# shayekh00/Knowledge_Distillation_for_Sensory_Substitution_in_Multimodal_Models

Measured on AMD Instinct MI355X. Metric: KD samples/sec/step (7B->0.5B, 336x336), higher is better.
Workload: dtype bf16; 1 GPU; c1: logit-based KD (LoCa, T=1), 7B->0.5B, 336x336; model=llava-onevision-qwen2-7b (teacher) -> 0.5b (student), global_batch=4, per_gpu_batch=4, seq_len=1536, image=336x336 (2 tiles, 1485 tokens), parallelism=dp1, teacher_lm_stream=bf16

## Files before the change

### include/kdstep.h

```cpp
#ifndef KDSTEP_H
#define KDSTEP_H

#include <stddef.h>
#include <stdint.h>

#ifdef __cplusplus
extern "C" {
#endif

typedef enum {
    KD_OK = 0,
    KD_ERR_SHAPE = 1,
    KD_ERR_DTYPE = 2,
    KD_ERR_ALIGN = 3,
    KD_ERR_ARCH = 4,
    KD_ERR_LABEL_RANGE = 5,
    KD_ERR_LAUNCH = 6,
    KD_ERR_ARG = 7,
    KD_ERR_WORKSPACE = 8
} kd_status;

int kd_abi_version(void);
const char* kd_last_error(void);
int kd_device_is_gfx950(int device);
// ... 79 lines not shown
    int32_t row_stats_top2;
    int32_t b_pretiled;
} kd_gemm_desc;

size_t kd_gemm_pretile_size(int N, int K, int glu);
int kd_gemm_pretile(const void* W, int64_t ldw, int N, int K, int glu, void* out, void* stream);
typedef struct kd_qkv_scatter {
    void* q; void* k; void* v;
    const float* cos_t; const float* sin_t;
    int32_t S, nq, nkv, hd, hdp;
} kd_qkv_scatter;

size_t kd_gemm_workspace_size(const kd_gemm_desc* desc);

int kd_gemm_plan(const kd_gemm_desc* desc, int32_t* variant, int32_t* split_k, int32_t* dp_tiles);

int kd_gemm(const kd_gemm_desc* desc, void* stream);

typedef struct {
    const void* q; const void* k; const void* v;
    void* o; float* lse;
    int32_t B, H, HKV, S, hd, hdp, causal;
} kd_attn_desc;
int kd_attn_fwd(const kd_attn_desc* desc, void* stream);

typedef struct {
    const void* q; const void* k; const void* v; const void* o; const void* dO;
    const float* lse; float* delta; float* dq; void* dk; void* dv;
    int32_t B, H, HKV, S, hd, hdp, causal;
    void* workspace; uint64_t workspace_bytes;
// ... 113 lines not shown
int kd_model_param_count(const kd_model_config* cfg);
int64_t kd_model_param_numel(const kd_model_config* cfg);
int kd_model_param_info(const kd_model_config* cfg, int index, char* name, int name_cap, int64_t* offset,
                        int64_t* numel, int64_t* rows, int64_t* cols);

int kd_anyres_batch_map(const int64_t* image_sizes_host, int B, int tiles, int32_t* map_host, int map_ld,
                        int32_t* len_host);

typedef struct kd_model kd_model;
int kd_model_create(const kd_model_config* cfg, const void* weights, float* grad, kd_model** out);
void kd_model_destroy(kd_model* m);
int kd_model_set_trainable(kd_model* m, int vision, int projector, int language);

int kd_model_set_residual_f32(kd_model* m, int vision, int language);

int64_t kd_model_fp8_scale_count(const kd_model* m);
int kd_model_quantize_fp8(const kd_model* m, void* q, float* scales, void* stream);
int kd_model_set_fp8(kd_model* m, const void* q, const float* scales);
typedef enum {
    KD_FP8_VISION = 1,
    KD_FP8_PROJECTOR = 2,
    KD_FP8_LM_ATTN = 4,
    KD_FP8_LM_MLP = 8,
    KD_FP8_LM_HEAD = 16,
    KD_FP8_ALL = 31
} kd_fp8_family;
int kd_model_set_fp8_families(kd_model* m, int families);

int kd_model_set_row_stats(kd_model* m, float* partials, int vs, float inv_t, int top2);

// ... 25 lines not shown
```

### knowledge_distillation_for_sensory_substitution_in_multimodal_models_amd/_native.py

```python
from __future__ import annotations

import ctypes as C
import os
from pathlib import Path

_PKG = Path(__file__).resolve().parent
LIB_PATH = Path(os.environ.get("KDSTEP_LIB", _PKG / "libkdstep.so"))
HEADER = _PKG.parent / "include" / "kdstep.h"

KD_OK = 0
ABI_VERSION = 9
STATUS_NAMES = {
    0: "KD_OK", 1: "KD_ERR_SHAPE", 2: "KD_ERR_DTYPE", 3: "KD_ERR_ALIGN", 4: "KD_ERR_ARCH",
    5: "KD_ERR_LABEL_RANGE", 6: "KD_ERR_LAUNCH", 7: "KD_ERR_ARG", 8: "KD_ERR_WORKSPACE",
}

KD_LOSS_NONE, KD_LOSS_LOCA, KD_LOSS_KL, KD_LOSS_KL_LOGTARGET = 0, 1, 2, 3


class KdLossParams(C.Structure):
    _fields_ = [
        ("variant", C.c_int32),
        ("temperature", C.c_float),
        ("alpha", C.c_float),
# ... 98 lines not shown
    "kd_last_error": (C.c_char_p, []),
    "kd_device_is_gfx950": (_i32, [_i32]),
    "kd_loss_workspace_size": (_sz, [_i32, _i32, _i32]),
    "kd_loss_fwd_bwd": (_i32, [_vp, _i64, _i32, _vp, _i64, _i32, _vp, _i32, _i32, KdLossParams,
                               _vp, _vp, _i64, _vp, _sz, _vp]),
    "kd_loss_check": (_i32, [_vp, _vp]),
    "kd_loss_student_stats": (_i32, [_vp, _i64, _i32, _i32, _f32, _vp, _vp]),
    "kd_gemm": (_i32, [C.POINTER(KdGemmDesc), _vp]),
    "kd_gemm_pretile_size": (_sz, [_i32, _i32, _i32]),
    "kd_gemm_pretile": (_i32, [_vp, _i64, _i32, _i32, _i32, _vp, _vp]),
    "kd_attn_fwd": (_i32, [C.POINTER(KdAttnDesc), _vp]),
    "kd_attn_bwd": (_i32, [C.POINTER(KdAttnBwdDesc), _vp]),
    "kd_attn_bwd_workspace_size": (C.c_size_t, [C.POINTER(KdAttnBwdDesc)]),
    "kd_gemm_workspace_size": (C.c_size_t, [C.POINTER(KdGemmDesc)]),
    "kd_gemm_plan": (_i32, [C.POINTER(KdGemmDesc), C.POINTER(_i32), C.POINTER(_i32), C.POINTER(_i32)]),
    "kd_norm_fwd": (_i32, [_i32, _vp, _i64, _vp, _vp, _vp, _i64, _vp, _vp, _i32, _i32, _f32, _i32, _vp]),
    "kd_norm_bwd_workspace_size": (_sz, [_i32, _i32]),
    "kd_norm_bwd": (_i32, [_i32, _vp, _i64, _vp, _vp, _i64, _vp, _vp, _vp, _i64, _i32, _vp, _vp, _i32, _vp, _sz,
                           _i32, _i32, _i32, _vp]),
    "kd_qkv_split": (_i32, [_vp, _i64, _vp, _vp, _vp, _vp, _vp, _i32, _i32, _i32, _i32, _i32, _i32, _vp]),
    "kd_qkv_merge": (_i32, [_vp, _vp, _vp, _vp, _i64, _vp, _vp, _i32, _i32, _i32, _i32, _i32, _i32, _vp]),
    "kd_swiglu_fwd": (_i32, [_vp, _i64, _vp, _i64, _i32, _i32, _vp]),
    "kd_swiglu_bwd": (_i32, [_vp, _i64, _vp, _i64, _vp, _i64, _i32, _i32, _vp]),
    "kd_act_bwd": (_i32, [_vp, _vp, _vp, _i64, _i32, _vp]),
    "kd_patchify": (_i32, [_vp, _i32, _vp, _i32, _i32, _i32, _i32, _vp]),
    "kd_embed_assemble": (_i32, [_vp, _vp, _vp, _vp, _vp, _vp, _i32, _i32, _i32, _vp, _vp]),
    "kd_image_src_map": (_i32, [_vp, _i32, _i32, _i64, _vp, _i32, _vp, _vp, _vp, _vp]),
    "kd_embed_bwd": (_i32, [_vp, _vp, _vp, _vp, _vp, _vp, _i32, _i32, _vp]),
    "kd_colsum": (_i32, [_vp, _i64, _i32, _i32, _vp, _i32, _vp]),
    "kd_row_group_mean": (_i32, [_vp, _i64, _i32, _i32, _i32, _vp, _vp]),
# ... 32 lines not shown
    "kd_gemv_gather_supported": (_i32, [_i32, _i32]),
    "kd_gemv_gather": (_i32, [_vp, _vp, _i64, _vp, _i32, _vp, _i32, _i32, _vp]),
    "kd_gemv_batch_gather": (_i32, [_vp, _i64, _i32, _vp, _i64, _vp, _i32, _vp, _i32, _i32, _vp]),
    "kd_gen_select_ids": (_i32, [_vp, _i64, _vp, _i32, _vp, _i32, _i32, _vp, _f32, _i32, _vp, _vp]),
    "kd_image_resize_u8": (_i32, [_vp, _i32, _i32, _vp, _i32, _i32, _vp, _sz, _vp]),
    "kd_anyres_tiles": (_i32, [_vp, _vp, _i32, _i32, _i32, _i32, _i32, _i32, _vp, _vp, _i32, _vp]),
    "kd_anyres_batch_map": (_i32, [_vp, _i32, _i32, _vp, _i32, _vp]),
    "kd_model_param_count": (_i32, [C.POINTER(KdModelConfig)]),
    "kd_model_param_numel": (_i64, [C.POINTER(KdModelConfig)]),
    "kd_model_param_info": (_i32, [C.POINTER(KdModelConfig), _i32, C.c_char_p, _i32, C.POINTER(_i64),
                                   C.POINTER(_i64), C.POINTER(_i64), C.POINTER(_i64)]),
    "kd_model_create": (_i32, [C.POINTER(KdModelConfig), _vp, _vp, C.POINTER(_vp)]),
    "kd_model_destroy": (None, [_vp]),
    "kd_model_set_trainable": (_i32, [_vp, _i32, _i32, _i32]),
    "kd_model_set_residual_f32": (_i32, [_vp, _i32, _i32]),
    "kd_model_fp8_scale_count": (_i64, [_vp]),
    "kd_model_quantize_fp8": (_i32, [_vp, _vp, _vp, _vp]),
    "kd_model_set_fp8": (_i32, [_vp, _vp, _vp]),
    "kd_model_set_fp8_families": (_i32, [_vp, _i32]),
    "kd_model_set_row_stats": (_i32, [_vp, _vp, _i32, _f32, _i32]),
    "kd_model_forward_workspace_size": (_sz, [_vp, _i32, _i32, _i32, _i32]),
    "kd_model_forward": (_i32, [_vp, _vp, _vp, _i32, _vp, _vp, _vp, _i32, _i32, _i32, _i32, _vp, _sz, _vp, _vp, _vp,
                                _vp, _vp, _vp, _vp]),
    "kd_model_backward_workspace_size": (_sz, [_vp, _i32, _i32, _i32]),
    "kd_model_backward": (_i32, [_vp, _vp, _vp, _vp, _vp, _vp, _i32, _i32, _i32, _vp, _vp, _vp, _sz, _vp, _vp,
                                 LAYER_CB, _vp]),
    "kd_timer_enable": (None, [_i32]),
    "kd_timer_count": (_i32, []),
    "kd_timer_read": (_i32, [_i32, C.c_char_p, _i32, C.POINTER(C.c_double), C.POINTER(_f32)]),
    "kd_timer_reset": (None, []),
# ... 40 lines not shown
```

### knowledge_distillation_for_sensory_substitution_in_multimodal_models_amd/csrc/abi.hip

```cpp
#include "common.h"
#include "launchers.h"
#include <cstring>

namespace kd {

static thread_local std::string g_last_error = "";

void set_error(const std::string& msg) { g_last_error = msg; }
int fail(int code, const std::string& msg) {
    g_last_error = msg;
    return code;
}

}

extern "C" {

int kd_abi_version(void) { return KD_ABI_VERSION; }

const char* kd_last_error(void) { return kd::g_last_error.c_str(); }

int kd_device_is_gfx950(int device) {
    hipDeviceProp_t prop;
    if (hipGetDeviceProperties(&prop, device) != hipSuccess) return 0;
// ... 13 lines not shown
int kd_loss_check(const void* workspace, void* stream) { return kd::kd_loss_check_impl(workspace, stream); }

int kd_loss_student_stats(const void* student_logits, int64_t ld_s, int V_s, int rows, float temperature,
                          float* stats_out, void* stream) {
    return kd::launch_kd_student_stats(student_logits, ld_s, V_s, rows, temperature, stats_out, stream);
}

int kd_gemm(const kd_gemm_desc* desc, void* stream) { return kd::gemm_timed(desc, stream); }
size_t kd_gemm_pretile_size(int N, int K, int glu) { return kd::gemm_pretile_size(N, K, glu); }
int kd_gemm_pretile(const void* W, int64_t ldw, int N, int K, int glu, void* out, void* stream) {
    return kd::launch_gemm_pretile(W, ldw, N, K, glu, out, stream);
}
size_t kd_gemm_workspace_size(const kd_gemm_desc* desc) { return kd::gemm_workspace_size(desc); }
int kd_gemm_plan(const kd_gemm_desc* desc, int32_t* variant, int32_t* split_k, int32_t* dp_tiles) {
    return kd::gemm_plan_query(desc, variant, split_k, dp_tiles);
}
int kd_attn_fwd(const kd_attn_desc* d, void* s) { return kd::launch_attn_fwd(d, s); }
int kd_attn_bwd(const kd_attn_bwd_desc* d, void* s) { return kd::launch_attn_bwd(d, s); }
size_t kd_attn_bwd_workspace_size(const kd_attn_bwd_desc* d) { return kd::attn_bwd_workspace_size(d); }
int kd_norm_fwd(int rms, const void* x, int64_t ldx, const void* w, const void* b, void* y, int64_t ldy, float* mean,
                float* rstd, int R, int D, float eps, int x_dtype, void* s) {
    KD_CHECK_ARG(x_dtype == KD_DTYPE_BF16 || x_dtype == KD_DTYPE_F32, "kd_norm_fwd: x_dtype");
    return kd::launch_norm_fwd(rms, x, ldx, w, b, y, ldy, mean, rstd, R, D, eps, s, x_dtype == KD_DTYPE_F32);
}
size_t kd_norm_bwd_workspace_size(int R, int D) { return kd::norm_bwd_ws(R, D); }
int kd_norm_bwd(int rms, const void* x, int64_t ldx, const void* w, const void* dy, int64_t lddy, const float* mean,
                const float* rstd, void* dx, int64_t lddx, int dx_accum, float* dw, float* db, int accum_w, void* ws,
                size_t wsb, int R, int D, int x_dtype, void* s) {
    KD_CHECK_ARG(x_dtype == KD_DTYPE_BF16 || x_dtype == KD_DTYPE_F32, "kd_norm_bwd: x_dtype");
    return kd::launch_norm_bwd(rms, x, ldx, w, dy, lddy, mean, rstd, dx, lddx, dx_accum, dw, db, accum_w, ws, wsb, R, D, s,
// ... 151 lines not shown
```

### knowledge_distillation_for_sensory_substitution_in_multimodal_models_amd/csrc/gemm.hip

```cpp
#include "common.h"

#include <cstring>
#include <type_traits>
#ifdef KD_AB_BUILD
#include <hipblaslt/hipblaslt.h>
#endif

namespace kd {
namespace {

constexpr int BM = 128, BN = 128, BK = 64, NTH = 256;
constexpr int TILE_BYTES = 128 * 64 * 2;
constexpr uint32_t OOB = 0x80000000u;

typedef __attribute__((address_space(3))) void lds_void_t;
typedef __attribute__((address_space(3))) bf16x4 lds_bf16x4_t;

struct GemmP {
    const bf16* A; const bf16* B; void* C;
    const void* bias; const bf16* resid; bf16* aux; const float* alpha_dev;
    int64_t lda, ldb, ldc, ldr, ld_aux;
    int M, N, K;
    float alpha;
    int c_f32, accumulate, bias_f32, act, res_mod;
// ... 1720 lines not shown
}
bool variant_known(int v) {
    const VariantInfo* i = variant_info(v);
#ifdef KD_AB_BUILD
    return i != nullptr;
#else
    return i && !i->ab;
#endif
}

bool sk_fits(int64_t tiles, int64_t nk, const kd_gemm_desc* d) {
    const int64_t dp = sk_dp_tiles(tiles, nk);
    return (tiles - dp) * nk >= 2 * SK_GRID && d->workspace && d->workspace_bytes >= sk_workspace_bytes(tiles - dp);
}

GemmPlan plan_gemm(const kd_gemm_desc* d, uint64_t ws_cap) {
    const int64_t M = d->M, N = d->N;
    const int64_t t256 = (int64_t)ceil_div(d->M, 256) * ceil_div(d->N, 256);
    const int64_t tiles[5] = {t256, (int64_t)ceil_div(d->M, 256) * ceil_div(d->N, 128),
                              (int64_t)ceil_div(d->M, 128) * ceil_div(d->N, 256), t256, t256};
    const bool kk = d->a_layout == KD_LAYOUT_K_MAJOR && d->b_layout == KD_LAYOUT_K_MAJOR;
    static const double step_c4[2][5] = {{0.8167, 0.5676, 0.5775, 0.7550, 0.7183}, {0.8016, 0.6139, 0.6026, 0.6942, 0.6876}};
    static const double fixed_c4[2][5] = {{8.830, 5.440, 5.343, 11.954, 5.888}, {9.291, 5.201, 5.162, 12.159, 8.442}};
    static const double step_c3[2][5] = {{0.7524, 0.5218, 0.5092, 0.6844, 0.7183}, {0.7375, 0.5501, 0.5469, 0.6022, 0.6876}};
    static const double fixed_c3[2][5] = {{5.253, 3.402, 3.414, 8.478, 5.888}, {5.885, 3.479, 3.398, 8.695, 8.442}};
    static const bool set3 = ab_knob("KD_PLAN_SET", 4) == 3;
    static const bool hybrid_on = ab_knob("KD_GEMM_HYBRID", 1) != 0;
    static const int split_cap = ab_knob("KD_SPLIT_CAP", 32);
    static const double split_pen = ab_knob("KD_SPLIT_PENALTY", 100) / 100.0;
    const double (&step_c)[2][5] = set3 ? step_c3 : step_c4;
    const double (&fixed_c)[2][5] = set3 ? fixed_c3 : fixed_c4;
    const double kBW = set3 ? 7.711e6 : 9.109e6;
    const double kSplitLaunch = set3 ? 5.623 : 6.499;
    constexpr bool kV9Auto = false;
    const double* step = step_c[kk ? 0 : 1];
    const double* fixed = fixed_c[kk ? 0 : 1];
    const int vcode[5] = {2, 3, 4, 16, 20};
    const int64_t nk = ceil_div(d->K, BK2);
    const VariantInfo* vi = variant_info(d->variant);
    const int fv = vi ? vi->cand : -1;
    const double out_e = (double)((d->c_dtype == KD_DTYPE_F32 ? 4 : 2) * (d->accumulate ? 2 : 1) +
                                  (d->residual ? (d->residual_dtype == KD_DTYPE_F32 ? 4 : 2) : 0) +
                                  (d->aux ? 2 : 0));
    const double out_b = (double)M * N * out_e;
    const int tbm[5] = {256, 256, 128, 256, 256}, tbn[5] = {256, 128, 256, 256, 256};
    GemmPlan best{fv >= 0 ? vcode[fv] : 2, 1, d->K, 0};
    double bt = 1e300;
    for (int v = 0; v < 5; ++v) {
        if (fv >= 0 && v != fv) continue;
        if (v == 4 && !kV9Auto && fv != 4) continue;
        for (int S = 1; S <= 32; ++S) {
// ... 49 lines not shown
    if (d->row_stats) return {Route::ROW_STATS, v8};
    if (d->act == KD_ACT_SWIGLU) {
        if (d->b_pretiled) return {Route::SWIGLU_PRETILED, v8};
        const bool sk = d->variant == 21 && sk_fits((int64_t)ceil_div(d->M, 256) * (d->N / 256), ceil_div(d->K, BK2), d);
        return {sk ? Route::SWIGLU_STREAMK : Route::SWIGLU, v8};
    }
    if (d->b_pretiled) return {Route::PRETILED, v8};
#ifdef KD_AB_BUILD
    if (d->variant == 30) return {Route::V8N, GemmPlan{30, 1, d->K, 0}};
#endif
    if (d->variant == 1 || !tiled_ok(d)) return {Route::V1, GemmPlan{1, 1, d->K, 0}};
    kd_gemm_desc d1 = *d;
    if (d->act == KD_ACT_DGELU_TANH || d->act == KD_ACT_DSWIGLU || d->qkv)
        d1.split_k = 1;
    return {Route::TILED, plan_gemm(&d1, d->workspace ? d->workspace_bytes : 0)};
}

GemmP make_params(const kd_gemm_desc* d) {
    GemmP p{};
    p.A = (const bf16*)d->A; p.B = (const bf16*)d->B; p.C = d->C;
    p.bias = d->bias; p.resid = (const bf16*)d->residual; p.aux = (bf16*)d->aux; p.alpha_dev = d->alpha_dev;
    p.lda = d->lda; p.ldb = d->ldb; p.ldc = d->ldc; p.ldr = d->ldr; p.ld_aux = d->ld_aux;
    p.M = d->M; p.N = d->N; p.K = d->K; p.alpha = d->alpha;
    p.c_f32 = d->c_dtype == KD_DTYPE_F32; p.accumulate = d->accumulate; p.bias_f32 = d->bias_dtype == KD_DTYPE_F32;
    p.act = d->act; p.res_mod = d->residual_row_mod;
    p.res_f32 = d->residual && d->residual_dtype == KD_DTYPE_F32;
    p.kchunk = d->K; p.gy = 1; p.rst_inv_t = 1.f;
    return p;
}

// ... 423 lines not shown
    }
    for (int i = n; i < GROUP_MAX; ++i) g.t0[i] = total;
    hipLaunchKernelGGL(k_gemm8_group, dim3((unsigned)total), dim3(NTH8), (gemm2_lds<256, 256>()), as_stream(stream_), g);
    KD_LAUNCH_CHECK("k_gemm8_group");
    return KD_OK;
}

int gemm_plan_query(const kd_gemm_desc* d, int32_t* var, int32_t* split, int32_t* dp) {
    KD_CHECK_ARG(d && var && split && dp, "gemm_plan: null pointer");
    KD_CHECK_SHAPE(d->M > 0 && d->N > 0 && d->K > 0, "gemm_plan: empty shape");
    const GemmPlan pl = gemm_route(d).plan;
    *var = pl.var; *split = pl.split; *dp = pl.dp_tiles;
    return KD_OK;
}

size_t gemm_workspace_size(const kd_gemm_desc* d) {
    if (!d || d->M <= 0 || d->N <= 0 || d->K <= 0 || d->variant == 1 || d->act == KD_ACT_SWIGLU) return 0;
    const GemmPlan pl = plan_gemm(d, ~0ull);
    if (pl.var == 21) return sk_workspace_bytes((int64_t)ceil_div(d->M, 256) * ceil_div(d->N, 256) - pl.dp_tiles);
    return pl.split > 1 ? (size_t)pl.split * d->M * d->N * 4 : 0;
}

}
```

### knowledge_distillation_for_sensory_substitution_in_multimodal_models_amd/csrc/launchers.h

```cpp
#pragma once
#include "common.h"

namespace kd {

int launch_kd_loss(const void* teacher, int64_t ld_t, int V_t, const void* student, int64_t ld_s,
                   int V_s, const int64_t* labels, int B, int L, kd_loss_params p, float* loss_out,
                   void* dlogits, int64_t ld_d, void* ws, size_t ws_bytes, void* stream);
size_t kd_loss_ws(int B, int L, int V);
int launch_kd_student_stats(const void* student, int64_t ld_s, int V_s, int rows, float temperature, float* out,
                            void* stream);
int kd_loss_check_impl(const void* ws, void* stream);
int launch_gemm(const kd_gemm_desc* d, void* stream);
int launch_gemm_group(const kd_gemm_desc* const* members, int n, void* stream);
bool gemm_group_member_ok(const kd_gemm_desc* d);
size_t gemm_workspace_size(const kd_gemm_desc* d);
size_t gemm_pretile_size(int N, int K, int glu);
int launch_gemm_pretile(const void* W, int64_t ldw, int N, int K, int glu, void* out, void* stream);
int gemm_plan_query(const kd_gemm_desc* d, int32_t* var, int32_t* split, int32_t* dp);
int launch_attn_fwd(const kd_attn_desc* d, void* stream);
int launch_attn_bwd(const kd_attn_bwd_desc* d, void* stream);
size_t attn_bwd_workspace_size(const kd_attn_bwd_desc* d);
int launch_norm_fwd(int rms, const void* x, int64_t ldx, const void* w, const void* b, void* y, int64_t ldy,
                    float* mean, float* rstd, int R, int D, float eps, void* stream, int x_f32 = 0);
size_t norm_bwd_ws(int R, int D);
int launch_norm_bwd(int rms, const void* x, int64_t ldx, const void* w, const void* dy, int64_t lddy, const float* mean,
                    const float* rstd, void* dx, int64_t lddx, int dx_accum, float* dw, float* db, int accum_w,
                    void* ws, size_t ws_bytes, int R, int D, void* stream, int x_f32 = 0, int dy_group = 0,
                    const void* dx_in = nullptr);
int launch_qkv_split(const void* qkv, int64_t ld, void* q, void* k, void* v, const float* cos_t, const float* sin_t,
                     int B, int S, int nq, int nkv, int hd, int hdp, void* stream);
int launch_qkv_merge(const float* dq, const void* dk, const void* dv, void* dqkv, int64_t ld, const float* cos_t,
                     const float* sin_t, int B, int S, int nq, int nkv, int hd, int hdp, void* stream);
int launch_swiglu_fwd(const void* gu, int64_t ldg, void* h, int64_t ldh, int M, int I, void* stream);
// ... 74 lines not shown
```

### knowledge_distillation_for_sensory_substitution_in_multimodal_models_amd/csrc/model.hip

```cpp
#include "common.h"
#include "launchers.h"

#include <algorithm>
#include <cmath>
#include <cstdlib>
#include <cstring>
#include <mutex>
#include <string>
#include <vector>

namespace kd {

namespace {
struct TimerRec {
    std::string key;
    double flops;
    hipEvent_t e0, e1;
};
std::mutex g_timer_mu;
std::vector<TimerRec> g_timer;
bool g_timer_on = false;
}

int gemm_timed(const kd_gemm_desc* d, void* stream) {
    if (!g_timer_on) return launch_gemm(d, stream);
    TimerRec r;
    const bool swiglu = d->act == KD_ACT_SWIGLU, f8 = d->ab_dtype == KD_DTYPE_FP8_E4M3;
    const bool dact = d->act == KD_ACT_DGELU_TANH || d->act == KD_ACT_DSWIGLU;
    r.key = swiglu ? std::string(f8 ? "gemm_f8_swiglu" : "gemm_kk_swiglu")
                   : (f8 ? std::string("gemm_f8") : std::string("gemm_") + (d->a_layout ? 'n' : 'k') + (d->b_layout ? 'n' : 'k') +
                                                        (dact ? "_dact" : ""));
    r.key += ":" + std::to_string(d->M) + "x" + std::to_string(d->N) + "x" + std::to_string(d->K) + ":" +
             (d->c_dtype == KD_DTYPE_F32 ? "f32" : "bf16") + (d->accumulate ? ":acc" : "");
    r.flops = 2.0 * d->M * d->N * d->K;
    (void)hipEventCreate(&r.e0);
    (void)hipEventCreate(&r.e1);
    (void)hipEventRecord(r.e0, as_stream(stream));
    const int st = launch_gemm(d, stream);
    (void)hipEventRecord(r.e1, as_stream(stream));
    std::lock_guard<std::mutex> g(g_timer_mu);
    g_timer.push_back(r);
    return st;
}

int gemm_group_timed(const kd_gemm_desc* const* ds, int n, void* stream) {
    if (!g_timer_on) return launch_gemm_group(ds, n, stream);
    TimerRec r;
    r.flops = 0;
// ... 124 lines not shown
enum LmField { LQW, LKW, LVW, LQB, LKB, LVB, LOW, LGW, LUW, LDW, LINW, LPOSTW, LNF };

}

}

struct kd_model {
    kd::Cfg C;
    std::vector<kd::Spec> specs;
    int64_t numel = 0;
    const kd::bf16* w = nullptr;
    float* g = nullptr;
    int train_vision = 0, train_projector = 0, train_language = 0;
    int lane_split_k = 0;
    int lane_group = 1, lane_v8_unsplit = 0;
    int rf32_v = 0, rf32_t = 0;
    std::vector<hipEvent_t> ev_pool;
    size_t ev_next = 0;
    const uint8_t* f8q = nullptr;
    const float* f8s = nullptr;
    std::vector<int64_t> soff;
    std::vector<int> fam;
    int f8_families = KD_FP8_ALL;
    float* rst = nullptr;
    int rst_vs = 0, rst_top2 = 0;
    float rst_inv_t = 1.f;
    int64_t n_scales = 0;
    int i_patch_w = 0, i_patch_b = 1, i_pos = 2, i_vis0 = 3, i_post_w, i_post_b, i_p1w, i_p1b, i_p2w, i_p2b, i_newline,
        i_embed, i_lm0, i_norm, i_head;

// ... 43 lines not shown
    const void* residual = nullptr;
    int64_t ldr = 0;
    void* aux = nullptr;
    int64_t ld_aux = 0;
    int residual_row_mod = 0;
    int accumulate = 0;
    int c_f32 = 0;
    int bias_f32 = 0;
    int split_k = 0;
    int res_f32 = 0;
    const kd_qkv_scatter* qkv = nullptr;
    float* row_stats = nullptr;
    int rs_vs = 0, rs_top2 = 0;
    float rs_inv_t = 1.f;
};

static const int g_split_default = ab_knob("KD_GEMM_SPLIT_K", 0);

int gemm(hipStream_t s, void* ws, int M, int N, int K, Op a, Op b, void* C, int64_t ldc, const GemmArgs& g) {
    kd_gemm_desc d;
    std::memset(&d, 0, sizeof(d));
    d.M = M; d.N = N; d.K = K;
    d.a_layout = a.layout; d.b_layout = b.layout;
    d.A = a.p; d.lda = a.ld; d.B = b.p; d.ldb = b.ld;
    d.C = C; d.ldc = ldc;
    d.c_dtype = g.c_f32 ? KD_DTYPE_F32 : KD_DTYPE_BF16;
    d.accumulate = g.accumulate;
    d.alpha = 1.f;
    d.bias = g.bias; d.bias_dtype = g.bias_f32 ? KD_DTYPE_F32 : KD_DTYPE_BF16;
    d.act = g.act;
    d.residual = g.residual; d.ldr = g.ldr;
    d.residual_dtype = g.res_f32 ? KD_DTYPE_F32 : KD_DTYPE_BF16;
    d.qkv = g.qkv;
    d.aux = g.aux; d.ld_aux = g.ld_aux;
    d.residual_row_mod = g.residual_row_mod;
    d.split_k = g.split_k ? g.split_k : g_split_default;
    if (d.split_k != 1 && ws) { d.workspace = ws; d.workspace_bytes = SPLITK_WS; }
    d.row_stats = g.row_stats; d.row_stats_vs = g.rs_vs; d.row_stats_inv_t = g.rs_inv_t; d.row_stats_top2 = g.rs_top2;
    return gemm_timed(&d, s);
}

static const bool g_fuse_dact = ab_knob("KD_FUSE_DACT", 1) != 0;
static bool fused_dact_ok(int64_t M, int64_t N) {
    return g_fuse_dact && M >= 128 && N >= 128 && N % 8 == 0 && M * N >= (int64_t)1 << 20;
}

#define KD_TRY(x)                    \
    do {                             \
        const int st__ = (x);        \
        if (st__ != KD_OK) return st__; \
    } while (0)

struct Lane {
    kd_model* m;
    hipStream_t main, lane;
    void* ws;
    void begin() {
        hipEvent_t e = m->event();
        (void)hipEventRecord(e, main);
        (void)hipStreamWaitEvent(lane, e, 0);
    }
    hipEvent_t end() {
        hipEvent_t e = m->event();
        (void)hipEventRecord(e, lane);
        return e;
    }
// ... 773 lines not shown
}

int kd_model_set_trainable(kd_model* m, int vision, int projector, int language) {
    KD_CHECK_ARG(m, "kd_model_set_trainable: null model");
    KD_CHECK_ARG(m->g || !(vision || projector || language), "kd_model_set_trainable: model has no grad buffer");
    m->train_vision = vision != 0;
    m->train_projector = projector != 0;
    m->train_language = language != 0;
    return KD_OK;
}

static bool fp8_stream_ok(bool f8, int fam, int rf32_v, int rf32_t) {
    return !f8 || ((!rf32_v || !(fam & KD_FP8_VISION)) && (!rf32_t || !(fam & (KD_FP8_LM_ATTN | KD_FP8_LM_MLP))));
}

int kd_model_set_residual_f32(kd_model* m, int vision, int language) {
    KD_CHECK_ARG(m, "kd_model_set_residual_f32: null model");
    KD_CHECK_ARG(fp8_stream_ok(m->f8q, m->f8_families, vision, language),
                 "kd_model_set_residual_f32: the tower's residual linears run in fp8 (bf16 residual only)");
    m->rf32_v = vision != 0;
    m->rf32_t = language != 0;
    return KD_OK;
}

int64_t kd_model_fp8_scale_count(const kd_model* m) { return m ? m->n_scales : -1; }

int kd_model_quantize_fp8(const kd_model* m, void* q, float* scales, void* stream) {
    KD_CHECK_ARG(m && q && scales, "kd_model_quantize_fp8: null pointer");
    KD_CHECK_ALIGN(q, 16, "kd_model_quantize_fp8: q must be 16-B aligned");
    for (size_t i = 0; i < m->specs.size(); ++i) {
// ... 45 lines not shown
    if (!m || B <= 0 || L <= 0 || n_tiles <= 0) return 0;
    return kd::plan_backward(m, B, L, n_tiles, nullptr).bytes;
}

int kd_model_forward(kd_model* m, const int64_t* ids, const void* pixels, int pixel_dtype, const int32_t* src,
                     const float* rope_cos, const float* rope_sin, int B, int L, int n_tiles, int save,
                     void* workspace, size_t workspace_bytes, void* hn, void* post_ln, void* logits,
                     void* const* kv_k, void* const* kv_v, int32_t* err, void* stream) {
    using namespace kd;
    KD_CHECK_ARG(m && ids && pixels && src && rope_cos && rope_sin && workspace && hn && err,
                 "kd_model_forward: null pointer");
    KD_CHECK_SHAPE(B > 0 && L > 0 && n_tiles > 0, "kd_model_forward: B, L, n_tiles must be positive");
    KD_CHECK_ARG(pixel_dtype == KD_DTYPE_BF16 || pixel_dtype == KD_DTYPE_F32, "kd_model_forward: pixel dtype");
    const FwdPlan P = plan_forward(m, B, L, n_tiles, save, workspace);
    KD_CHECK_ARG(workspace_bytes >= P.bytes, "kd_model_forward: workspace too small");
    const kd_model_config& c = m->C.c;
    hipStream_t s = as_stream(stream);
    const int NI = n_tiles, M = B * L, H = c.t_hidden;
    KD_TRY(vision_forward(m, P, pixels, pixel_dtype, NI, save, post_ln, s));
    {
        const int NT = NI * m->C.np(), D = c.v_hidden;
        GemmArgs g;
        g.bias = m->W(m->i_p1b);
        g.act = c.projector_act;
        g.aux = save ? P.ppre : nullptr;
        g.ld_aux = H;
        KD_TRY(lin(m, P, s, NT, H, D, P.x_vis_bf, D, m->i_p1w, P.z, H, g));
        GemmArgs g2;
        g2.bias = m->W(m->i_p2b);
        KD_TRY(lin(m, P, s, NT, H, H, P.z, H, m->i_p2w, P.feats, H, g2));
// ... 10 lines not shown
    return KD_OK;
}

int kd_model_backward(kd_model* m, const void* fwd_workspace, const int64_t* ids, const int32_t* src,
                      const float* rope_cos, const float* rope_sin, int B, int L, int n_tiles, const void* dhn,
                      const void* dpost, void* workspace, size_t workspace_bytes, void* stream, void* wgrad_stream,
                      kd_layer_cb on_layer_done, void* user) {
    using namespace kd;
    KD_CHECK_ARG(m && fwd_workspace && ids && src && rope_cos && rope_sin && dhn && workspace && wgrad_stream,
                 "kd_model_backward: null pointer");
    KD_CHECK_ARG(m->g, "kd_model_backward: the model has no grad buffer");
    KD_CHECK_SHAPE(B > 0 && L > 0 && n_tiles > 0, "kd_model_backward: B, L, n_tiles must be positive");
    const FwdPlan F = plan_forward(m, B, L, n_tiles, 1, const_cast<void*>(fwd_workspace));
    const BwdPlan P = plan_backward(m, B, L, n_tiles, workspace);
    KD_CHECK_ARG(workspace_bytes >= P.bytes, "kd_model_backward: workspace too small");
    const kd_model_config& c = m->C.c;
    hipStream_t s = as_stream(stream);
    Lane lane{m, s, as_stream(wgrad_stream), P.splitk_lane};
    hipEvent_t entry = m->event();
    (void)hipEventRecord(entry, lane.lane);
    const int NI = n_tiles, NT = NI * m->C.np(), M = B * L, H = c.t_hidden, D = c.v_hidden;
    const bf16* demb = nullptr;
    KD_TRY(lm_backward(m, F, P, rope_cos, rope_sin, B, L, dhn, lane, s, on_layer_done, user, &demb));
    wait(s, entry);
    const bool need_vision = m->train_vision != 0;
    KD_TRY(launch_embed_bwd(ids, src, demb, m->train_language ? m->G(m->i_embed) : nullptr, P.dfeats,
                            m->train_projector ? m->G(m->i_newline) : nullptr, M, H, s));
    {
        GemmArgs g0;
        KD_TRY(gemm(s, P.splitk_main, NT, H, H, km(P.dfeats, H), mn(m->W(m->i_p2w), H), P.dz, H, g0));
// ... 58 lines not shown
```

### knowledge_distillation_for_sensory_substitution_in_multimodal_models_amd/kd_module.py

```python
from __future__ import annotations

import contextlib
import inspect


import torch
import torch.nn as nn

from . import ops
from .dp import BackwardMarks, GradSync
from .modeling import (STREAM_PRIORITY_HIGH, STUDENT_05B, TEACHER_7B, LlavaOnevisionModel, real_width_config,
                       tiny_config)

try:
    import pytorch_lightning as _pl
    _Base = _pl.LightningModule
except Exception:
    class _Base(nn.Module):
        def __init__(self):
            super().__init__()
            self.logged = {}

        def log(self, name, value, **kw):
            self.logged[name] = value
# ... 168 lines not shown
        self.processor = processor
        self.model_name_student, self.model_name_teacher = model_name_student, model_name_teacher
        self.loss_group_size = loss_group_size
        self.accumulate_grad_batches = None if accumulate_grad_batches is None else int(accumulate_grad_batches)
        dev = _device()
        small = model_name_student not in _HUB_NAMES
        self.student_model = LlavaOnevisionModel(MODEL_CONFIGS[model_name_student], dev, trainable=True,
                                                 seed=seed_student, cpu_rng=small)
        self.teacher_model = None
        if self.uses_teacher:
            self.teacher_model = LlavaOnevisionModel(MODEL_CONFIGS[model_name_teacher], dev, trainable=False,
                                                     seed=seed_teacher, cpu_rng=small)
        if state_dict is not None:
            self.load_kd_state_dict(state_dict)
        self.config = self.student_model.cfg
        self._anchor = nn.Parameter(torch.zeros((), device=dev))
        self._stu_stream = torch.cuda.Stream(device=dev, priority=STREAM_PRIORITY_HIGH)
        self._opt_stream = self._stu_stream
        self.concurrent_student = True
        self._opt_done = torch.cuda.Event()
        self._opt_pending = False
        self._bwd_stream = self._stu_stream
        self._bwd_done = torch.cuda.Event()
        self._bwd_pending = False
        self.student_model.P.grad_fence = self._grad_fence
        self._ctx = None
        self._errors = _ErrorWatch(dev)
        self._errors.bind(self.student_model, self.teacher_model)
        self.keep_logits = False
        self.fuse_row_stats = False
# ... 261 lines not shown
    def kd_state_dict(self):
        if self._opt_pending:
            torch.cuda.current_stream().wait_event(self._opt_done)
        sd = {f"{self.ckpt_student_prefix}{k}": v for k, v in self.student_model.P.state_dict().items()}
        if self.teacher_model is not None:
            sd.update({f"teacher_model.{k}": v for k, v in self.teacher_model.P.state_dict().items()})
        return sd

    def load_kd_state_dict(self, sd):
        self.student_model.P.load_state_dict(sd, prefix=self.ckpt_student_prefix)
        if self.teacher_model is not None and any(k.startswith("teacher_model.") for k in sd):
            self.teacher_model.P.load_state_dict(sd, prefix="teacher_model.")
            if getattr(self.teacher_model, "fp8", False):
                self.teacher_model.enable_fp8(self.teacher_model.fp8_families)

    def load_hf_weights(self, student: dict | None = None, teacher: dict | None = None, strict: bool = True):
        if student is not None:
            self.student_model.load_hf_state_dict(student, strict=strict)
        if teacher is not None:
            if self.teacher_model is None:
                raise ValueError(f"{type(self).__name__} has no teacher")
            self.teacher_model.load_hf_state_dict(teacher, strict=strict)

    def _hparams(self):
        return {"model_name_student": self.model_name_student, "model_name_teacher": self.model_name_teacher,
                "learning_rate": self.learning_rate, "phase": self.phase, **self._run_hparams()}

    def _run_hparams(self):
        return {"loss_group_size": self.loss_group_size, "accumulate_grad_batches": self.accumulate_grad_batches,
                "teacher_fp8": getattr(self, "teacher_fp8", False),
# ... 104 lines not shown
```

### knowledge_distillation_for_sensory_substitution_in_multimodal_models_amd/modeling.py

```python
from __future__ import annotations

import ctypes as C
from dataclasses import dataclass, field

import numpy as np
import torch

from . import _native as NV
from . import anyres
from . import ops

IMAGE_TOKEN_ID = 151646


@dataclass(frozen=True)
class VisionConfig:
    hidden: int = 1152
    inter: int = 4304
    layers: int = 26
    heads: int = 16
    patch: int = 14
    image: int = 384
    eps: float = 1e-6

# ... 337 lines not shown
        self._ws = {}
        self.err = torch.zeros(1, dtype=torch.int32, device=self.device)
        self._train = [trainable] * 3
        self.wlane = WgradLane(self.device) if (trainable and self.device.type == "cuda") else None
        self._ncfg = native_config(cfg)
        if NV.lib().kd_model_param_numel(C.byref(self._ncfg)) != self.P.numel:
            raise RuntimeError("flat parameter layout differs from the library's (kd_model_param_info)")
        h = C.c_void_p()
        NV.call("kd_model_create", C.byref(self._ncfg), self.P.flat.data_ptr(),
                self.P.grad.data_ptr() if trainable else None, C.byref(h))
        self._h = h
        self.fp8 = False
        self.residual_f32 = (False, False)
        self.fp8_families = 0
        self.lm_stream_f32 = False
        self.set_residual_f32(*self._default_streams())

    def set_residual_f32(self, vision: bool, language: bool):
        NV.call("kd_model_set_residual_f32", self._h, int(vision), int(language))
        self.residual_f32 = (bool(vision), bool(language))
        self._ws = {}

    def __del__(self):
        h = getattr(self, "_h", None)
        if h is None or not h.value:
            return
        try:
            NV.lib().kd_model_destroy(h)
        except Exception:
            return
        self._h = None

    def set_trainable(self, vision: bool, projector: bool, language: bool):
        self._train = [bool(vision), bool(projector), bool(language)]
        NV.call("kd_model_set_trainable", self._h, *map(int, self._train))

# ... 170 lines not shown
```

### knowledge_distillation_for_sensory_substitution_in_multimodal_models_amd/ops.py

```python
from __future__ import annotations

import contextlib
import ctypes as C

import torch

from . import _native as NV

_WS: dict = {}


class KernelTimer:

    @property
    def enabled(self):
        return getattr(self, "_on", False)

    @enabled.setter
    def enabled(self, on):
        self._on = bool(on)
        NV.lib().kd_timer_enable(int(self._on))

    def reset(self):
        NV.lib().kd_timer_reset()
# ... 222 lines not shown
        _set_pretiled(d, b_pretiled, N, K, False)
    NV.call("kd_gemm", C.byref(d), _stream())
    return q, k, v


def gemm_plan(a: torch.Tensor, b: torch.Tensor, out: torch.Tensor | None = None, *, bias=None, act=None,
              residual=None, aux=None, alpha: float = 1.0, alpha_dev=None, accumulate: bool = False,
              out_dtype=torch.bfloat16, residual_row_mod: int = 0, variant: int = 0, split_k: int = 0):
    d = _gemm_desc(a, b, out, bias, act, residual, aux, alpha, alpha_dev, accumulate, out_dtype, residual_row_mod,
                   variant, split_k)[0]
    v, s_, dp = C.c_int32(), C.c_int32(), C.c_int32()
    NV.call("kd_gemm_plan", C.byref(d), C.byref(v), C.byref(s_), C.byref(dp))
    return v.value, s_.value, dp.value


_SPLIT_DEFAULT = [0]


@contextlib.contextmanager
def gemm_split_default(split_k: int):
    prev = _SPLIT_DEFAULT[0]
    _SPLIT_DEFAULT[0] = int(split_k)
    try:
        yield
    finally:
        _SPLIT_DEFAULT[0] = prev


def gemm(a: torch.Tensor, b: torch.Tensor, out: torch.Tensor | None = None, *, bias=None, act=None,
         residual=None, aux=None, alpha: float = 1.0, alpha_dev=None, accumulate: bool = False,
# ... 578 lines not shown
```

Measured before the change: 30.00 samples/s.

## Add CU-time GEMM planning objective for student training GEMMs

Adds a second GEMM planner objective that picks tile variant and split-K by total CU time rather than single-kernel latency, using the existing analytic cost model. The student model enables it by default for saved forward and backward passes, on the idea that student GEMMs run alongside the teacher and other streams, so CU occupancy matters more than isolated latency. This risks slower individual GEMMs when there is little concurrent work, and it relies on the accuracy of the cost model.

```diff
diff --git a/include/kdstep.h b/include/kdstep.h
--- a/include/kdstep.h
+++ b/include/kdstep.h
@@ -117,6 +117,11 @@
 size_t kd_gemm_workspace_size(const kd_gemm_desc* desc);
 
 int kd_gemm_plan(const kd_gemm_desc* desc, int32_t* variant, int32_t* split_k, int32_t* dp_tiles);
+
+typedef enum { KD_PLAN_LATENCY = 0, KD_PLAN_CU_TIME = 1 } kd_plan_objective;
+
+int kd_gemm_plan_objective(const kd_gemm_desc* desc, int objective, int32_t* variant, int32_t* split_k,
+                           int32_t* dp_tiles, double* latency_us, double* cu_us);
 
 int kd_gemm(const kd_gemm_desc* desc, void* stream);
 
@@ -260,6 +265,8 @@
 
 int kd_model_set_residual_f32(kd_model* m, int vision, int language);
 
+int kd_model_set_plan_objective(kd_model* m, int objective);
+
 int64_t kd_model_fp8_scale_count(const kd_model* m);
 int kd_model_quantize_fp8(const kd_model* m, void* q, float* scales, void* stream);
 int kd_model_set_fp8(kd_model* m, const void* q, const float* scales);
diff --git a/knowledge_distillation_for_sensory_substitution_in_multimodal_models_amd/_native.py b/knowledge_distillation_for_sensory_substitution_in_multimodal_models_amd/_native.py
--- a/knowledge_distillation_for_sensory_substitution_in_multimodal_models_amd/_native.py
+++ b/knowledge_distillation_for_sensory_substitution_in_multimodal_models_amd/_native.py
@@ -136,6 +136,8 @@
     "kd_attn_bwd_workspace_size": (C.c_size_t, [C.POINTER(KdAttnBwdDesc)]),
     "kd_gemm_workspace_size": (C.c_size_t, [C.POINTER(KdGemmDesc)]),
     "kd_gemm_plan": (_i32, [C.POINTER(KdGemmDesc), C.POINTER(_i32), C.POINTER(_i32), C.POINTER(_i32)]),
+    "kd_gemm_plan_objective": (_i32, [C.POINTER(KdGemmDesc), _i32, C.POINTER(_i32), C.POINTER(_i32), C.POINTER(_i32),
+                                      C.POINTER(C.c_double), C.POINTER(C.c_double)]),
     "kd_norm_fwd": (_i32, [_i32, _vp, _i64, _vp, _vp, _vp, _i64, _vp, _vp, _i32, _i32, _f32, _i32, _vp]),
     "kd_norm_bwd_workspace_size": (_sz, [_i32, _i32]),
     "kd_norm_bwd": (_i32, [_i32, _vp, _i64, _vp, _vp, _i64, _vp, _vp, _vp, _i64, _i32, _vp, _vp, _i32, _vp, _sz,
@@ -198,6 +200,7 @@
     "kd_model_destroy": (None, [_vp]),
     "kd_model_set_trainable": (_i32, [_vp, _i32, _i32, _i32]),
     "kd_model_set_residual_f32": (_i32, [_vp, _i32, _i32]),
+    "kd_model_set_plan_objective": (_i32, [_vp, _i32]),
     "kd_model_fp8_scale_count": (_i64, [_vp]),
     "kd_model_quantize_fp8": (_i32, [_vp, _vp, _vp, _vp]),
     "kd_model_set_fp8": (_i32, [_vp, _vp, _vp]),
diff --git a/knowledge_distillation_for_sensory_substitution_in_multimodal_models_amd/csrc/abi.hip b/knowledge_distillation_for_sensory_substitution_in_multimodal_models_amd/csrc/abi.hip
--- a/knowledge_distillation_for_sensory_substitution_in_multimodal_models_amd/csrc/abi.hip
+++ b/knowledge_distillation_for_sensory_substitution_in_multimodal_models_amd/csrc/abi.hip
@@ -51,6 +51,16 @@
 size_t kd_gemm_workspace_size(const kd_gemm_desc* desc) { return kd::gemm_workspace_size(desc); }
 int kd_gemm_plan(const kd_gemm_desc* desc, int32_t* variant, int32_t* split_k, int32_t* dp_tiles) {
     return kd::gemm_plan_query(desc, variant, split_k, dp_tiles);
+}
+int kd_gemm_plan_objective(const kd_gemm_desc* desc, int objective, int32_t* variant, int32_t* split_k, int32_t* dp_tiles,
+                           double* latency_us, double* cu_us) {
+    KD_CHECK_ARG(variant && split_k && dp_tiles && latency_us && cu_us, "kd_gemm_plan_objective: null pointer");
+    kd::GemmObjectivePlan pl;
+    const int st = kd::gemm_plan_objective_query(desc, objective, &pl);
+    if (st != KD_OK) return st;
+    *variant = pl.variant; *split_k = pl.split_k; *dp_tiles = pl.dp_tiles;
+    *latency_us = pl.latency_us; *cu_us = pl.cu_us;
+    return KD_OK;
 }
 int kd_attn_fwd(const kd_attn_desc* d, void* s) { return kd::launch_attn_fwd(d, s); }
 int kd_attn_bwd(const kd_attn_bwd_desc* d, void* s) { return kd::launch_attn_bwd(d, s); }
diff --git a/knowledge_distillation_for_sensory_substitution_in_multimodal_models_amd/csrc/gemm.hip b/knowledge_distillation_for_sensory_substitution_in_multimodal_models_amd/csrc/gemm.hip
--- a/knowledge_distillation_for_sensory_substitution_in_multimodal_models_amd/csrc/gemm.hip
+++ b/knowledge_distillation_for_sensory_substitution_in_multimodal_models_amd/csrc/gemm.hip
@@ -1,4 +1,5 @@
 #include "common.h"
+#include "launchers.h"
 
 #include <cstring>
 #include <type_traits>
@@ -1758,11 +1759,14 @@
     return (tiles - dp) * nk >= 2 * SK_GRID && d->workspace && d->workspace_bytes >= sk_workspace_bytes(tiles - dp);
 }
 
-GemmPlan plan_gemm(const kd_gemm_desc* d, uint64_t ws_cap) {
-    const int64_t M = d->M, N = d->N;
-    const int64_t t256 = (int64_t)ceil_div(d->M, 256) * ceil_div(d->N, 256);
-    const int64_t tiles[5] = {t256, (int64_t)ceil_div(d->M, 256) * ceil_div(d->N, 128),
-                              (int64_t)ceil_div(d->M, 128) * ceil_div(d->N, 256), t256, t256};
+struct PlanModel {
+    const double* step;
+    const double* fixed;
+    double kBW, kSplitLaunch, split_pen;
+    int split_cap;
+    bool hybrid_on;
+};
+PlanModel plan_model(const kd_gemm_desc* d) {
     const bool kk = d->a_layout == KD_LAYOUT_K_MAJOR && d->b_layout == KD_LAYOUT_K_MAJOR;
     static const double step_c4[2][5] = {{0.8167, 0.5676, 0.5775, 0.7550, 0.7183}, {0.8016, 0.6139, 0.6026, 0.6942, 0.6876}};
     static const double fixed_c4[2][5] = {{8.830, 5.440, 5.343, 11.954, 5.888}, {9.291, 5.201, 5.162, 12.159, 8.442}};
@@ -1776,9 +1780,20 @@
     const double (&fixed_c)[2][5] = set3 ? fixed_c3 : fixed_c4;
     const double kBW = set3 ? 7.711e6 : 9.109e6;
     const double kSplitLaunch = set3 ? 5.623 : 6.499;
+    return {step_c[kk ? 0 : 1], fixed_c[kk ? 0 : 1], kBW, kSplitLaunch, split_pen, split_cap, hybrid_on};
+}
+
+GemmPlan plan_gemm(const kd_gemm_desc* d, uint64_t ws_cap) {
+    const int64_t M = d->M, N = d->N;
+    const int64_t t256 = (int64_t)ceil_div(d->M, 256) * ceil_div(d->N, 256);
+    const int64_t tiles[5] = {t256, (int64_t)ceil_div(d->M, 256) * ceil_div(d->N, 128),
+                              (int64_t)ceil_div(d->M, 128) * ceil_div(d->N, 256), t256, t256};
+    const PlanModel pm = plan_model(d);
+    const double *step = pm.step, *fixed = pm.fixed;
+    const double kBW = pm.kBW, kSplitLaunch = pm.kSplitLaunch, split_pen = pm.split_pen;
+    const int split_cap = pm.split_cap;
+    const bool hybrid_on = pm.hybrid_on;
     constexpr bool kV9Auto = false;
-    const double* step = step_c[kk ? 0 : 1];
-    const double* fixed = fixed_c[kk ? 0 : 1];
     const int vcode[5] = {2, 3, 4, 16, 20};
     const int64_t nk = ceil_div(d->K, BK2);
     const VariantInfo* vi = variant_info(d->variant);
@@ -1858,6 +1873,55 @@
     if (d->act == KD_ACT_DGELU_TANH || d->act == KD_ACT_DSWIGLU || d->qkv)
         d1.split_k = 1;
     return {Route::TILED, plan_gemm(&d1, d->workspace ? d->workspace_bytes : 0)};
+}
+
+struct PlanCost { double latency_us, cu_us; };
+PlanCost plan_cost(const kd_gemm_desc* d, const GemmPlan& pl) {
+    const int v = pl.var == 2 ? 0 : pl.var == 3 ? 1 : pl.var == 4 ? 2 : pl.var == 16 ? 3 : pl.var == 20 ? 4 : -1;
+    if (v < 0) return {0, 0};
+    const int tbm[5] = {256, 256, 128, 256, 256}, tbn[5] = {256, 128, 256, 256, 256};
+    const PlanModel pm = plan_model(d);
+    const int64_t tiles = (int64_t)ceil_div(d->M, tbm[v]) * ceil_div(d->N, tbn[v]);
+    const int64_t nk = ceil_div(d->K, BK2), S = pl.split, kcs = S > 1 ? ceil_div(pl.kchunk, BK2) : nk;
+    const double whole = (double)nk * pm.step[v] + pm.fixed[v], part = (double)kcs * pm.step[v] + pm.fixed[v];
+    const double out_e = (double)((d->c_dtype == KD_DTYPE_F32 ? 4 : 2) * (d->accumulate ? 2 : 1) +
+                                  (d->residual ? (d->residual_dtype == KD_DTYPE_F32 ? 4 : 2) : 0) + (d->aux ? 2 : 0));
+    const int64_t dp = S > 1 ? pl.dp_tiles : 0, tail = tiles - dp;
+    const double elems = dp ? (double)tail * tbm[v] * tbn[v] : (double)d->M * d->N;
+    const double fold = S > 1 ? ((double)S * elems * 8 * pm.split_pen + elems * out_e) / pm.kBW + (dp ? 2 : 1) * pm.kSplitLaunch : 0;
+    const double lat = (double)(dp / 256) * whole + (double)((tail * S + 255) / 256) * part + fold;
+    const double cu = ((double)dp * whole + (double)tail * S * part) / 256 + fold;
+    return {lat, cu};
+}
+
+constexpr double kCuMargin = 0.05;
+
+GemmObjectivePlan plan_gemm_objective(const kd_gemm_desc* d, int objective) {
+    const GemmRoute r0 = gemm_route(d);
+    const PlanCost c0 = plan_cost(d, r0.plan);
+    const GemmObjectivePlan keep{r0.plan.var, r0.plan.split, r0.plan.dp_tiles, c0.latency_us, c0.cu_us, false};
+    const int fv = d->variant;
+    if (objective == 0 || r0.route != Route::TILED || !(fv == 0 || fv == 2 || fv == 3 || fv == 4 || fv == 16)) return keep;
+    GemmObjectivePlan best = keep;
+    bool found = false;
+    for (int code : {2, 3, 4, 16}) {
+        if (fv != 0 && code != fv) continue;
+        kd_gemm_desc df = *d;
+        df.variant = code;
+        df.split_k = d->split_k > 1 ? d->split_k : 1;
+        const GemmRoute r = gemm_route(&df);
+        if (r.route != Route::TILED || r.plan.var != code) continue;
+        const PlanCost c = plan_cost(&df, r.plan);
+        if (!found || c.cu_us < best.cu_us) {
+            best = GemmObjectivePlan{r.plan.var, r.plan.split, r.plan.dp_tiles, c.latency_us, c.cu_us, true};
+            found = true;
+        }
+    }
+    if (!found || best.cu_us > c0.cu_us) return keep;
+    if (best.variant == keep.variant && best.split_k == keep.split_k && best.dp_tiles == keep.dp_tiles) return keep;
+    const bool lat_is_candidate = r0.plan.dp_tiles == 0 && (r0.plan.split == 1 || d->split_k > 1);
+    if (lat_is_candidate && best.cu_us > c0.cu_us * (1.0 - kCuMargin)) return keep;
+    return best;
 }
 
 GemmP make_params(const kd_gemm_desc* d) {
@@ -2311,6 +2375,14 @@
     return KD_OK;
 }
 
+int gemm_plan_objective_query(const kd_gemm_desc* d, int objective, GemmObjectivePlan* out) {
+    KD_CHECK_ARG(d && out, "gemm_plan_objective: null pointer");
+    KD_CHECK_ARG(objective == KD_PLAN_LATENCY || objective == KD_PLAN_CU_TIME, "gemm_plan_objective: objective must be 0 or 1");
+    KD_CHECK_SHAPE(d->M > 0 && d->N > 0 && d->K > 0, "gemm_plan_objective: empty shape");
+    *out = plan_gemm_objective(d, objective);
+    return KD_OK;
+}
+
 size_t gemm_workspace_size(const kd_gemm_desc* d) {
     if (!d || d->M <= 0 || d->N <= 0 || d->K <= 0 || d->variant == 1 || d->act == KD_ACT_SWIGLU) return 0;
     const GemmPlan pl = plan_gemm(d, ~0ull);
diff --git a/knowledge_distillation_for_sensory_substitution_in_multimodal_models_amd/csrc/launchers.h b/knowledge_distillation_for_sensory_substitution_in_multimodal_models_amd/csrc/launchers.h
--- a/knowledge_distillation_for_sensory_substitution_in_multimodal_models_amd/csrc/launchers.h
+++ b/knowledge_distillation_for_sensory_substitution_in_multimodal_models_amd/csrc/launchers.h
@@ -17,6 +17,8 @@
 size_t gemm_pretile_size(int N, int K, int glu);
 int launch_gemm_pretile(const void* W, int64_t ldw, int N, int K, int glu, void* out, void* stream);
 int gemm_plan_query(const kd_gemm_desc* d, int32_t* var, int32_t* split, int32_t* dp);
+struct GemmObjectivePlan { int variant, split_k, dp_tiles; double latency_us, cu_us; bool forced; };
+int gemm_plan_objective_query(const kd_gemm_desc* d, int objective, GemmObjectivePlan* out);
 int launch_attn_fwd(const kd_attn_desc* d, void* stream);
 int launch_attn_bwd(const kd_attn_bwd_desc* d, void* stream);
 size_t attn_bwd_workspace_size(const kd_attn_bwd_desc* d);
diff --git a/knowledge_distillation_for_sensory_substitution_in_multimodal_models_amd/csrc/model.hip b/knowledge_distillation_for_sensory_substitution_in_multimodal_models_amd/csrc/model.hip
--- a/knowledge_distillation_for_sensory_substitution_in_multimodal_models_amd/csrc/model.hip
+++ b/knowledge_distillation_for_sensory_substitution_in_multimodal_models_amd/csrc/model.hip
@@ -20,6 +20,15 @@
 std::mutex g_timer_mu;
 std::vector<TimerRec> g_timer;
 bool g_timer_on = false;
+
+thread_local int t_plan_objective = KD_PLAN_LATENCY;
+struct PlanScope {
+    const int prev = t_plan_objective;
+    explicit PlanScope(int objective) { t_plan_objective = objective; }
+    ~PlanScope() { t_plan_objective = prev; }
+    PlanScope(const PlanScope&) = delete;
+    PlanScope& operator=(const PlanScope&) = delete;
+};
 }
 
 int gemm_timed(const kd_gemm_desc* d, void* stream) {
@@ -32,6 +41,10 @@
                                                         (dact ? "_dact" : ""));
     r.key += ":" + std::to_string(d->M) + "x" + std::to_string(d->N) + "x" + std::to_string(d->K) + ":" +
              (d->c_dtype == KD_DTYPE_F32 ? "f32" : "bf16") + (d->accumulate ? ":acc" : "");
+    if (t_plan_objective == KD_PLAN_CU_TIME) {
+        int32_t var = 0, split = 1, dp = 0;
+        if (gemm_plan_query(d, &var, &split, &dp) == KD_OK && split > 1) r.key += ":s" + std::to_string(split);
+    }
     r.flops = 2.0 * d->M * d->N * d->K;
     (void)hipEventCreate(&r.e0);
     (void)hipEventCreate(&r.e1);
@@ -186,6 +199,7 @@
     int train_vision = 0, train_projector = 0, train_language = 0;
     int lane_split_k = 0;
     int lane_group = 1, lane_v8_unsplit = 0;
+    int plan_objective = KD_PLAN_LATENCY;
     int rf32_v = 0, rf32_t = 0;
     std::vector<hipEvent_t> ev_pool;
     size_t ev_next = 0;
@@ -259,6 +273,12 @@
     int rs_vs = 0, rs_top2 = 0;
     float rs_inv_t = 1.f;
 };
+
+#define KD_TRY(x)                    \
+    do {                             \
+        const int st__ = (x);        \
+        if (st__ != KD_OK) return st__; \
+    } while (0)
 
 static const int g_split_default = ab_knob("KD_GEMM_SPLIT_K", 0);
 
@@ -282,6 +302,11 @@
     d.split_k = g.split_k ? g.split_k : g_split_default;
     if (d.split_k != 1 && ws) { d.workspace = ws; d.workspace_bytes = SPLITK_WS; }
     d.row_stats = g.row_stats; d.row_stats_vs = g.rs_vs; d.row_stats_inv_t = g.rs_inv_t; d.row_stats_top2 = g.rs_top2;
+    if (t_plan_objective == KD_PLAN_CU_TIME) {
+        GemmObjectivePlan pl;
+        KD_TRY(gemm_plan_objective_query(&d, KD_PLAN_CU_TIME, &pl));
+        if (pl.forced) { d.variant = pl.variant; d.split_k = pl.split_k; }
+    }
     return gemm_timed(&d, s);
 }
 
@@ -289,12 +314,6 @@
 static bool fused_dact_ok(int64_t M, int64_t N) {
     return g_fuse_dact && M >= 128 && N >= 128 && N % 8 == 0 && M * N >= (int64_t)1 << 20;
 }
-
-#define KD_TRY(x)                    \
-    do {                             \
-        const int st__ = (x);        \
-        if (st__ != KD_OK) return st__; \
-    } while (0)
 
 struct Lane {
     kd_model* m;
@@ -1098,6 +1117,14 @@
     return !f8 || ((!rf32_v || !(fam & KD_FP8_VISION)) && (!rf32_t || !(fam & (KD_FP8_LM_ATTN | KD_FP8_LM_MLP))));
 }
 
+int kd_model_set_plan_objective(kd_model* m, int objective) {
+    KD_CHECK_ARG(m, "kd_model_set_plan_objective: null model");
+    KD_CHECK_ARG(objective == KD_PLAN_LATENCY || objective == KD_PLAN_CU_TIME,
+                 "kd_model_set_plan_objective: objective must be KD_PLAN_LATENCY or KD_PLAN_CU_TIME");
+    m->plan_objective = objective;
+    return KD_OK;
+}
+
 int kd_model_set_residual_f32(kd_model* m, int vision, int language) {
     KD_CHECK_ARG(m, "kd_model_set_residual_f32: null model");
     KD_CHECK_ARG(fp8_stream_ok(m->f8q, m->f8_families, vision, language),
@@ -1173,6 +1200,7 @@
     KD_CHECK_ARG(pixel_dtype == KD_DTYPE_BF16 || pixel_dtype == KD_DTYPE_F32, "kd_model_forward: pixel dtype");
     const FwdPlan P = plan_forward(m, B, L, n_tiles, save, workspace);
     KD_CHECK_ARG(workspace_bytes >= P.bytes, "kd_model_forward: workspace too small");
+    const PlanScope plan_scope(save ? m->plan_objective : KD_PLAN_LATENCY);
     const kd_model_config& c = m->C.c;
     hipStream_t s = as_stream(stream);
     const int NI = n_tiles, M = B * L, H = c.t_hidden;
@@ -1213,6 +1241,7 @@
     const FwdPlan F = plan_forward(m, B, L, n_tiles, 1, const_cast<void*>(fwd_workspace));
     const BwdPlan P = plan_backward(m, B, L, n_tiles, workspace);
     KD_CHECK_ARG(workspace_bytes >= P.bytes, "kd_model_backward: workspace too small");
+    const PlanScope plan_scope(m->plan_objective);
     const kd_model_config& c = m->C.c;
     hipStream_t s = as_stream(stream);
     Lane lane{m, s, as_stream(wgrad_stream), P.splitk_lane};
diff --git a/knowledge_distillation_for_sensory_substitution_in_multimodal_models_amd/kd_module.py b/knowledge_distillation_for_sensory_substitution_in_multimodal_models_amd/kd_module.py
--- a/knowledge_distillation_for_sensory_substitution_in_multimodal_models_amd/kd_module.py
+++ b/knowledge_distillation_for_sensory_substitution_in_multimodal_models_amd/kd_module.py
@@ -206,6 +206,7 @@
         if state_dict is not None:
             self.load_kd_state_dict(state_dict)
         self.config = self.student_model.cfg
+        self.cu_time_plans = True
         self._anchor = nn.Parameter(torch.zeros((), device=dev))
         self._stu_stream = torch.cuda.Stream(device=dev, priority=STREAM_PRIORITY_HIGH)
         self._opt_stream = self._stu_stream
@@ -497,6 +498,14 @@
             if getattr(self.teacher_model, "fp8", False):
                 self.teacher_model.enable_fp8(self.teacher_model.fp8_families)
 
+    @property
+    def cu_time_plans(self) -> bool:
+        return self.student_model.plan_objective == 1
+
+    @cu_time_plans.setter
+    def cu_time_plans(self, on: bool):
+        self.student_model.set_plan_objective(1 if on else 0)
+
     def load_hf_weights(self, student: dict | None = None, teacher: dict | None = None, strict: bool = True):
         if student is not None:
             self.student_model.load_hf_state_dict(student, strict=strict)
diff --git a/knowledge_distillation_for_sensory_substitution_in_multimodal_models_amd/modeling.py b/knowledge_distillation_for_sensory_substitution_in_multimodal_models_amd/modeling.py
--- a/knowledge_distillation_for_sensory_substitution_in_multimodal_models_amd/modeling.py
+++ b/knowledge_distillation_for_sensory_substitution_in_multimodal_models_amd/modeling.py
@@ -375,12 +375,17 @@
         self.residual_f32 = (False, False)
         self.fp8_families = 0
         self.lm_stream_f32 = False
+        self.plan_objective = 0
         self.set_residual_f32(*self._default_streams())
 
     def set_residual_f32(self, vision: bool, language: bool):
         NV.call("kd_model_set_residual_f32", self._h, int(vision), int(language))
         self.residual_f32 = (bool(vision), bool(language))
         self._ws = {}
+
+    def set_plan_objective(self, objective: int):
+        NV.call("kd_model_set_plan_objective", self._h, int(objective))
+        self.plan_objective = int(objective)
 
     def __del__(self):
         h = getattr(self, "_h", None)
diff --git a/knowledge_distillation_for_sensory_substitution_in_multimodal_models_amd/ops.py b/knowledge_distillation_for_sensory_substitution_in_multimodal_models_amd/ops.py
--- a/knowledge_distillation_for_sensory_substitution_in_multimodal_models_amd/ops.py
+++ b/knowledge_distillation_for_sensory_substitution_in_multimodal_models_amd/ops.py
@@ -260,6 +260,17 @@
     return v.value, s_.value, dp.value
 
 
+def gemm_plan_objective(objective: int, a: torch.Tensor, b: torch.Tensor, out: torch.Tensor | None = None, **kw):
+    kw = {"bias": None, "act": None, "residual": None, "aux": None, "alpha": 1.0, "alpha_dev": None, "accumulate": False,
+          "out_dtype": torch.bfloat16, "residual_row_mod": 0, "variant": 0, "split_k": 0, **kw}
+    d = _gemm_desc(a, b, out, kw["bias"], kw["act"], kw["residual"], kw["aux"], kw["alpha"], kw["alpha_dev"],
+                   kw["accumulate"], kw["out_dtype"], kw["residual_row_mod"], kw["variant"], kw["split_k"])[0]
+    v, s_, dp, lat, cu = C.c_int32(), C.c_int32(), C.c_int32(), C.c_double(), C.c_double()
+    NV.call("kd_gemm_plan_objective", C.byref(d), int(objective), C.byref(v), C.byref(s_), C.byref(dp), C.byref(lat),
+            C.byref(cu))
+    return v.value, s_.value, dp.value, lat.value, cu.value
+
+
 _SPLIT_DEFAULT = [0]
 
 
```

New measurement: 30.70 samples/s (median of 6 runs). 1.02x the previous value.
